# Zydak/Vulkan-Path-Tracer

Hardware: AMD Instinct MI355X
Metric: Msamples/s at 1920x1080 (higher is better)
Workload: dtype f32; 1 GPU; cornell_1080p_d8; scene=CornellBox (12 triangles, emissive quad 50), black env, width=1920, height=1080, max_depth=8, samples_per_frame=1, batches_per_gpu=14 x 904 frames, partition=rows y % N == rank, one ncclGather at the end, base_seed=1

## Files before the change

### vulkan-path-tracer_amd/_build.py

```python
import os
import subprocess
import sys

HERE = os.path.dirname(os.path.abspath(__file__))
CSRC = os.path.join(HERE, "csrc")
LIB = os.path.join(HERE, "libvpt_hip.so")
LIB_LAB = os.path.join(HERE, "libvpt_hip_lab.so")
SOURCES = ["kernels_whole.hip", "kernels_finish.hip", "kernels_bounce.hip", "kernels_aux.hip", "kernels_trace.hip", "kernels_stream.hip", "kernels_media.hip", "kernels_post.hip",
           "api_context.hip", "api_scene.hip", "api_render.hip", "api_post.hip", "api_comm.hip", "bvh_build.cpp"]
LAB_SOURCES = ["kernels_lab_r1.hip", "api_lab.hip"]
HEADERS = ["kernels_lut.hip", "device_types.hpp", "path_plan.hpp", "scene_prep.hpp", "grid_prep.hpp", "denoise.hpp", "temporal.hpp", "kernels.hpp", "api_ctx.hpp", "shading.hpp", "traverse.hpp", "bvh_build.hpp", "bvh_refit.hpp", "volume.hpp", "atmosphere.hpp", "wave.hpp", "shade_core.hpp", "vote.hpp", "slab.hpp", "whole_refill.hpp", "whole_args.hpp", "camera.hpp", "camera_cull.hpp",
           os.path.join("..", "..", "include", "vpt.h"), os.path.join("..", "..", "include", "vpt_lab.h"), os.path.join("..", "..", "include", "vpt_fp32.h")]
FLAGS = ["--offload-arch=gfx950", "-O3", "-std=c++17", "-fPIC", "-ffp-contract=off", "-fno-fast-math",
         "-fhip-fp32-correctly-rounded-divide-sqrt", "-Wno-unused-result", "-Wno-pass-failed"]
EXTRA_FLAGS = {f: ["-fno-slp-vectorize"] for f in ("kernels_trace.hip", "kernels_stream.hip", "kernels_media.hip", "kernels_whole.hip", "kernels_finish.hip", "kernels_bounce.hip", "kernels_aux.hip", "kernels_lab_r1.hip")}
EXTRA_FLAGS.update({f: ["-Os"] for f in ("api_context.hip", "api_scene.hip", "api_render.hip", "api_post.hip", "api_comm.hip")})
EXTRA_FLAGS["bvh_build.cpp"] = ["-O2"]
EXTRA_FLAGS["kernels_post.hip"] = ["-Xarch_host", "-Os"]


def hipcc():
    for c in (os.environ.get("HIPCC"), "/opt/rocm/bin/hipcc", "hipcc"):
        if c and (os.path.isabs(c) and os.path.exists(c) or not os.path.isabs(c)):
            return c
    raise RuntimeError("hipcc not found")


def _sources(lab):
    return SOURCES + (LAB_SOURCES if lab else [])


def source_id(defines=("-DVPT_LAB=0",)):
    import hashlib
    h = hashlib.sha256()
# ... 63 lines not shown
```

### vulkan-path-tracer_amd/csrc/api_context.hip

```cpp
#include <cmath>

#include "api_ctx.hpp"

using namespace vpt::api;

namespace {

bool media_on(const vpt_ctx* c) { return !c->volumes.empty() || c->dsc.atm_on; }
void free_path_buffers(Lane& L) {
    destroy_graph(L);
    if (L.ps_block) (void)hipFree(L.ps_block);
    L.ps_block = nullptr;
    if (L.ps_legacy) (void)hipFree(L.ps_legacy);
    L.ps_legacy = nullptr;
    for (int i = 0; i < 2; i++) { if (L.queue[i]) (void)hipFree(L.queue[i]); L.queue[i] = nullptr; }
    if (L.cqueue) (void)hipFree(L.cqueue);
    L.cqueue = nullptr;
    if (L.ss_block) (void)hipFree(L.ss_block);
    L.ss_block = nullptr;
    if (L.media_block) (void)hipFree(L.media_block);
    L.media_block = nullptr; L.ms = MediaState{}; L.media_frames = 0;
    for (uint32_t k = 0; k < kShadeClasses; k++) { if (L.class_queue[k]) (void)hipFree(L.class_queue[k]); L.class_queue[k] = nullptr; }
    if (L.cls_q) (void)hipFree(L.cls_q);
    L.cls_q = nullptr;
// ... 409 lines not shown
    free_render_buffers(c);
    if (c->d_launch_off) (void)hipFree(c->d_launch_off);
    if (c->d_volumes) (void)hipFree(c->d_volumes);
    for (DensityGrid& g : c->grids) { (void)hipFree((void*)g.values); (void)hipFree((void*)g.block_max); (void)hipFree((void*)g.bricks); }
    if (c->d_grids) (void)hipFree(c->d_grids);
    for (hipEvent_t e : c->ev_pool) (void)hipEventDestroy(e);
    lane_destroy(c->main);
    delete c;
}

const char* vpt_last_error(const vpt_ctx* c) { return c ? c->err.c_str() : "null context"; }

int vpt_set_camera(vpt_ctx* c, const float* vi, const float* pi) {
    if (!c || !vi || !pi) return VPT_ERR_INVALID_ARGUMENT;
    memcpy(c->P.view_inv, vi, 64); memcpy(c->P.proj_inv, pi, 64);
    c->state_gen++;
    reset_accum(c, true);
    return VPT_OK;
}

int vpt_set_params(vpt_ctx* c, const vpt_params* p) {
    if (!c || !p) return VPT_ERR_INVALID_ARGUMENT;
    if (p->samples_per_frame == 0 || p->samples_per_frame > 0xffffffu) return fail(c, VPT_ERR_INVALID_ARGUMENT, "samples_per_frame must be >= 1");
    if (p->max_depth == 0 || p->max_depth > 1000000u) return fail(c, VPT_ERR_INVALID_ARGUMENT, "max_depth must be in [1, 1000000]");
    if (p->screen_chunk_count == 0 || p->screen_chunk_count > 64) return fail(c, VPT_ERR_INVALID_ARGUMENT, "screen_chunk_count must be in [1, 64]");
    if (p->screen_chunk_count != 1 && c->P.shard_count != 1) return fail(c, VPT_ERR_UNSUPPORTED, "split-screen dispatch needs the whole image in one context (shard_count == 1): its first dispatch copies pixels across rows");
    {
        vpt_params same = *p; same.max_samples = c->params.max_samples;
        if (p->max_samples != c->params.max_samples && memcmp(&same, &c->params, sizeof(vpt_params)) == 0) { c->params.max_samples = p->max_samples; return VPT_OK; }
    }
    { int rd = drain(c); if (rd) return rd; }
    c->state_gen++;
    const bool flags_changed = c->params.flags != p->flags;
    c->dsc.strict_hits = (p->flags & VPT_FLAG_LOCAL_HITS) ? 1u : 0u;
    c->params = *p;
    sync_params(c);
    reset_accum(c);
    if (flags_changed && c->has_scene) {
        HIPCHK(c, hipSetDevice(c->cfg.device));
        int rc2 = refresh_material_tables(c); if (rc2) return rc2;
    }
    return VPT_OK;
}

int vpt_set_base_seed(vpt_ctx* c, uint32_t base_seed) {
    if (!c) return VPT_ERR_INVALID_ARGUMENT;
    { int rd = drain(c); if (rd) return rd; }
// ... 54 lines not shown
```

### vulkan-path-tracer_amd/csrc/api_render.hip

```cpp
#include "api_ctx.hpp"

using namespace vpt::api;
using plan::Kind;

namespace {


uint32_t split_dispatch_slots(const RenderParams& P, uint32_t dispatch) {
    const uint32_t S = P.split, ch = dispatch % (S * S), cx = ch % S, cy = ch / S;
    const uint32_t lw = cx < P.width ? (P.width - cx + S - 1) / S : 0, lh = cy < P.height ? (P.height - cy + S - 1) / S : 0;
    return lw * lh;
}
uint32_t batch_slots(const RenderParams& P, uint32_t frames, uint32_t dispatch_base) {
    if (P.split <= 1) return frames * P.shard_pixels;
    uint32_t n = 0;
    for (uint32_t k = 0; k < frames; k++) n += split_dispatch_slots(P, dispatch_base + k);
    return n;
}
int decide_batch(vpt_ctx* c, const Lane& L, const plan::Facts& f, uint32_t frames, uint32_t dispatch_base, bool capturing, plan::Schedule& sd) {
    if (frames == 0 || frames > L.frames_alloc) return fail(c, VPT_ERR_DEVICE, "internal: batch larger than the path buffers");
    sd = plan::decide(f, frames, L.frames_alloc, L.resident_alloc, batch_slots(c->P, frames, dispatch_base), &L != &c->main, capturing);
    return sd.err != VPT_OK ? fail(c, sd.err, sd.msg) : VPT_OK;
}
PathState part_state(const vpt_ctx* c, const Lane& L, uint32_t first_frame) {
    PathState ps = L.ps;
    const size_t at = (size_t)first_frame * c->P.shard_pixels;
    ps.ACC += at; ps.M += at; ps.maniso += at;
    return ps;
}
void resolve_part(vpt_ctx* c, Lane& L, const BatchState& b, uint32_t i, hipStream_t on) {
    const uint32_t first = b.sd.parts.first[i];
    const uint32_t* guard = plan::runs_fused(b.sd.kind) ? &L.ctr->alive3[b.k3] : plan::runs_streams(b.sd.kind) ? &L.sctr->alive[b.parity].v : &L.ctr->ray_count[b.parity];
    TIMED(c, on, VPT_K_RESOLVE, launch_resolve(on, c->P, part_state(c, L, first), c->image, b.sd.parts.first[i + 1] - first, b.dispatch_base + first, guard));
}
int batch_begin(vpt_ctx* c, Lane& L, const plan::Schedule& sd, uint32_t frames, uint32_t dispatch_base, Grids grids, BatchState& b) {
    hipStream_t s = L.stream;
    b = BatchState{};
    b.frames = frames; b.dispatch_base = dispatch_base; b.sd = sd;
    b.primary_grid = grids.primary; b.tail_grid = grids.tail;
    c->spill_dirty = true;
    const uint32_t n_slots = batch_slots(c->P, frames, dispatch_base);
    if (c->P.split > 1) {
        std::vector<uint32_t> off(frames + 1, 0u);
        for (uint32_t k = 0; k < frames; k++) off[k + 1] = off[k] + split_dispatch_slots(c->P, dispatch_base + k);
        HIPCHK(c, hipMemcpyAsync(c->d_launch_off, off.data(), off.size() * 4, hipMemcpyHostToDevice, s));
        HIPCHK(c, hipStreamSynchronize(s));
    }
    b.n_slots = n_slots;
    b.n_first = sd.regen ? sd.resident * c->P.shard_pixels : n_slots;
    b.count = c->cfg.count_traversal != 0;
    if (sd.kind == Kind::MediaStreams) {
        int rl = ensure_media_buffers(c, L); if (rl != VPT_OK) return rl;
        if (frames > L.media_frames) return fail(c, VPT_ERR_DEVICE, "internal: media batch larger than the media streams");
    }
    if (sd.kind == Kind::StagedR1) { int rl = ensure_legacy_buffers(c, L); if (rl != VPT_OK) return rl; }
    if (sd.kind == Kind::StreamsSorted) { int rl = ensure_sorted_buffers(c, L); if (rl != VPT_OK) return rl; }
    b.min_bounces = (uint64_t)c->P.max_depth * c->P.samples_per_frame;
    b.iter_cap = (b.min_bounces * 4ull + 1024ull) * ((frames + sd.resident - 1) / sd.resident);
    if (n_slots == 0) return VPT_OK;
    HIPCHK(c, hipMemsetAsync(L.ctr, 0, offsetof(Counters, stat_closest), s));
    const DeviceScene dsc = lane_scene(c, L);
    if (sd.kind == Kind::Whole) {
        b.parity = 1; b.k3 = 1; b.iter = 1;
        const cull::Packed rect = cull::pack(whole_cull_rect(c));
        for (uint32_t i = 0; i < sd.parts.n; i++) {
            const uint32_t first = sd.parts.first[i], n_part = sd.parts.n > 1u ? (sd.parts.first[i + 1] - first) * c->P.shard_pixels : n_slots;
            const uint32_t grid = std::max(1u, std::min<uint32_t>((uint32_t)std::min(c->whole_blocks, b.primary_grid), (n_part + 255u) / 256u));
            const uint32_t n_waves = grid * 4u, rounds = ((n_part + 63u) / 64u) / n_waves, mode = c->lab_whole_sched >> 4;
            const uint32_t static_rounds = (mode == 0u || mode == 3u) ? std::min(rounds, 1u) : mode == 1u ? (rounds >= 2u ? rounds - 1u : 0u) : rounds / 2u;
            if (i) HIPCHK(c, hipMemsetAsync(&L.ctr->extend_head, 0, 4, s));
            TIMED(c, s, VPT_K_PRIMARY, launch_whole(s, grid, b.count, dsc, c->P, part_state(c, L, first), L.ctr, n_part, dispatch_base + first, c->scene_plain, static_rounds, std::max(1u, c->lab_whole_sched & 15u) | (mode == 3u ? 0x100u : 0u), rect.x, rect.y));
            if (i + 1u < sd.parts.n) {
                HIPCHK(c, hipEventRecord(L.ev_shade, s));
                HIPCHK(c, hipStreamWaitEvent(L.stream2, L.ev_shade, 0));
                resolve_part(c, L, b, i, L.stream2);
            }
        }
    } else if (sd.kind == Kind::Fused) {
        TIMED(c, s, VPT_K_PRIMARY, launch_bounce(s, (uint32_t)b.primary_grid, c->lds_scene, b.count, true, dsc, c->P, L.ps, L.ss, nullptr, L.queue[1], L.ctr, 0u, b.n_first, dispatch_base, 0u, c->scene_plain));
        b.parity = 1; b.k3 = 1; b.iter = 1;
    } else if (plan::runs_streams(sd.kind)) {
        TIMED(c, s, VPT_K_PRIMARY, launch_raygen_stream(s, c->P, L.ps, L.ss, L.queue[0], b.n_first, dispatch_base, sd.kind == Kind::MediaStreams));
        launch_stream_begin(s, L.sctr, b.n_first, n_slots);
        b.parity = 0;
    } else {
#if VPT_LAB
        TIMED(c, s, VPT_K_PRIMARY, launch_raygen(s, c->P, L.ps, L.queue[0], L.ctr, n_slots, dispatch_base));
#endif
        b.parity = 0;
    }
    return VPT_OK;
}

int batch_bounces(vpt_ctx* c, Lane& L, BatchState& b, uint32_t bounces) {
// ... 509 lines not shown
```

### vulkan-path-tracer_amd/csrc/device_types.hpp

```cpp
#pragma once
#include <hip/hip_runtime.h>
#include <stdint.h>

#include "../../include/vpt.h"
#include "../../include/vpt_fp32.h"

namespace vpt {

using vptfp::V2;
using vptfp::V3;
using vptfp::V4;

struct BvhNode {
    float origin[3];
    float step_x;
    uint32_t lo[3];
    uint32_t hi[3];
    float step_y, step_z;
    int32_t child[4];
    __host__ __device__ void set_step(int axis, uint32_t biased_exponent) {
        uint32_t bits = biased_exponent << 23; float f; __builtin_memcpy(&f, &bits, 4);
        (axis == 0 ? step_x : axis == 1 ? step_y : step_z) = f;
    }
};
// ... 184 lines not shown
    uint32_t* SHI;
    float4* PE;
    float4* PS;
    float4* PL;
    float4* PT;
    float4* SKO;
    float4* SKD;
    float4* LTO;
    float4* LTD;
    unsigned char* vis_sky;
    unsigned char* vis_light;
    uint32_t cap;
};

struct MediaState {
    float4* MS;
    float4* MP[10];
};

struct alignas(256) HotWord {
    uint32_t v;
    uint32_t pad[63];
};
constexpr uint32_t kShadeMiss = 0, kShadePlain = 1, kShadeTextured = 2, kShadeGlass = 3, kShadeEmissive = 4, kShadeClasses = 5;
constexpr int kShadeAny = -1;

struct StreamCounters {
    HotWord queue_len[2];
    HotWord alive[2];
    HotWord pend_len, sky_len, light_len;
    HotWord extend_head, shade_head, sky_head, light_head;
    HotWord finish_head;
    HotWord class_len[kShadeClasses];
    HotWord class_head[kShadeClasses];
    uint32_t class_active[kShadeClasses];
    uint32_t class_exact[kShadeClasses];
    uint32_t class_base[kShadeClasses];
    uint32_t classify_done;
    uint32_t refill_next, refill_total;
    uint32_t refill_entry, refill_first, refill_count;
};

constexpr uint32_t kAppendChunk = 256;
constexpr uint32_t kAppendExactBelow = 1u << 21;
constexpr uint32_t kFusedExactBelow = kAppendExactBelow;

// ... 22 lines not shown
```

### vulkan-path-tracer_amd/csrc/kernels.hpp

```cpp
#pragma once
#include "device_types.hpp"
#include "denoise.hpp"
#include "temporal.hpp"
#include "../../include/vpt_lab.h"
#ifndef VPT_LAB
#define VPT_LAB 0
#endif

namespace vpt {

void launch_bounce(hipStream_t s, uint32_t blocks, bool lds_scene, bool count, bool first, const DeviceScene& sc, const RenderParams& P,
                   const PathState& ps, const StreamState& ss, const uint32_t* queue, uint32_t* queue_next, Counters* ctr, uint32_t parity, uint32_t n_slots,
                   uint32_t dispatch_base, uint32_t k3, bool plain = false);
int bounce_blocks_per_cu(bool lds_scene, const DeviceScene& sc, bool plain = false);
void launch_whole(hipStream_t s, uint32_t blocks, bool count, const DeviceScene& sc, const RenderParams& P, const PathState& ps, Counters* ctr, uint32_t n_slots,
                  uint32_t dispatch_base, bool plain, uint32_t static_rounds, uint32_t chunk_tiles, uint32_t cull_x, uint32_t cull_y);
int whole_blocks_per_cu(const DeviceScene& sc, bool plain);
void launch_finish(hipStream_t s, uint32_t blocks, bool count, const DeviceScene& sc, const RenderParams& P, const PathState& ps, const StreamState& ss, const uint32_t* queue,
                   StreamCounters* sctr, Counters* ctr, uint32_t parity);
int finish_blocks_per_cu(const DeviceScene& sc);
void launch_resolve(hipStream_t s, const RenderParams& P, const PathState& ps, float* image, uint32_t frames, uint32_t frame_base, const uint32_t* guard);
struct FirstHitArgs {
    const vpt_ray* rays; vpt_hit* hits; uint32_t n;
    uint32_t mode, frame;
    float* depth; uint4* ids; float4* normal; float4* albedo;
    float4* pick; uint32_t pixel;
};
void launch_first_hit(hipStream_t s, uint32_t blocks, const DeviceScene& sc, const RenderParams& P, const FirstHitArgs& a);
void launch_trace_rays(hipStream_t s, uint32_t blocks, const DeviceScene& sc, const vpt_ray* rays, uint32_t n, vpt_hit* hits);
void launch_read_density_grid(hipStream_t s, const DensityGrid& g, const int32_t* ijk, uint32_t n, float* out);
void launch_scatter_rows(hipStream_t s, const float* gathered, float* full, uint32_t w, uint32_t h, uint32_t shard_count, uint32_t stride_px);
void launch_precompute_materials(hipStream_t s, const DeviceScene& sc, uint32_t flags, MatResolved* out, uint32_t n);
void launch_precompute_tri_ng(hipStream_t s, const DeviceScene& sc, float4* out);
void launch_precompute_tri_shade(hipStream_t s, const DeviceScene& sc, float4* out);
void launch_precompute_emissive(hipStream_t s, const DeviceScene& sc, EmissiveTri* out, uint32_t total);
void launch_retransform_tris(hipStream_t s, const DeviceScene& sc, uint32_t total_tris, uint32_t n_inst, uint32_t first, uint32_t count, const float* xf, BvhTri* out, uint32_t* words);
void launch_refit_level(hipStream_t s, const DeviceScene& sc, const uint32_t* order, uint32_t begin, uint32_t end, const BvhTri* tris, float pad, float* boxes, BvhNode* nodes_out, BvhNodeWide* wide_out);
size_t traverse_lds_bytes(const DeviceScene& sc, bool lds_scene, int stack_rows);
size_t stack_overflow_bytes(uint32_t blocks);
// ... 94 lines not shown
```

### vulkan-path-tracer_amd/csrc/kernels_whole.hip

```cpp
#include "kernels.hpp"
#include "traverse.hpp"
#include "wave.hpp"
#include "shade_core.hpp"
#include "whole_refill.hpp"
#include "whole_args.hpp"
#include "camera_cull.hpp"

namespace vpt {

#define VPT_KERNARG __attribute__((address_space(4)))
template <> struct OneSampleFrames<VPT_KERNARG WholeParams> { static constexpr bool value = true; };

template <class Pm, class Ps>
__device__ __forceinline__ V3 whole_finish(const Pm& P, const Ps& ps, uint32_t slot, V3 E, V3 thr_prev, V3 light_prev, const ShadeOut& o) {
    const V3 light = light_prev + path_contribution(E, thr_prev, o.cflags, P.max_luminance);
    if (o.terminated) ps.ACC[slot] = finite3(light) ? f4(v3s(0.0f) + light, 0.0f) : make_float4(0.0f, 0.0f, 0.0f, 0.0f);
    return light;
}
template <bool COUNT, bool STRICT, bool PLAIN>
__global__ __launch_bounds__(kTraverseBlock, 3) void k_whole(WholeLaunch wl) {
    const WholeArgs& a = wl.a;
    const DeviceScene sc = a.sc;
    const RenderParams P = a.P;
    Counters* const ctr = a.ctr;
    extern __shared__ __align__(16) unsigned char smem[];
    const TravStackT<kWholeStackRows> stack = make_stack<kWholeStackRows>(smem, sc.stack_overflow);
    float4* lds_nodes = reinterpret_cast<float4*>(smem + kWholeStackRows * kTraverseBlock * 4);
    float4* lds_tris = lds_nodes + sc.node_count * 8;
    __shared__ CameraBlock cam;
    if (threadIdx.x == 0u) fill_camera_block(cam, P.view_inv, P.proj_inv, P.width, P.height, P.focus_distance, P.dof_strength);
    const VPT_KERNARG WholeArgs* ka = (const VPT_KERNARG WholeArgs*)__builtin_amdgcn_kernarg_segment_ptr();
    stage_scene<true>(sc, lds_nodes, lds_tris);
    constexpr uint32_t kWaves = kTraverseBlock / 64u;
    __shared__ uint32_t r_slot[kWaves][128], r_prim[kWaves][128], r_inst[kWaves][128];
    __shared__ float r_t[kWaves][128], r_u[kWaves][128], r_v[kWaves][128];
    __shared__ float4 r_ra[kWaves][128], r_rb[kWaves][128], r_rt[kWaves][128];
    __shared__ uint32_t f_slot[kWaves][refill::kTile], f_rng[kWaves][refill::kTile];
    __shared__ float f_ox[kWaves][refill::kTile], f_oy[kWaves][refill::kTile], f_oz[kWaves][refill::kTile];
    __shared__ float f_dx[kWaves][refill::kTile], f_dy[kWaves][refill::kTile], f_dz[kWaves][refill::kTile];
    const uint32_t wave = __builtin_amdgcn_readfirstlane(threadIdx.x >> 6);
    const refill::Shape shape{a.n_slots, gridDim.x * kWaves, a.static_rounds, a.chunk_tiles};
    refill::Cursor cur = refill::make_cursor(shape, blockIdx.x * kWaves + wave);
    refill::Fresh fresh = refill::make_fresh();
    uint32_t hit_head = 0u, hit_count = 0u;
    TravStats st, sst; st.nodes = 0; st.tris = 0; sst.nodes = 0; sst.tris = 0;
    uint32_t w_paths = 0u, w_rays = 0u, w_hits0 = 0u, w_alive0 = 0u, w_rays0 = 0u, w_parked = 0u;
#if VPT_LAB
    uint32_t w_culled = 0u;
#endif
    bool has_ray = false;
    uint32_t slot = 0u, rng_s = 0u, depth = 0u;
    bool in_medium = false;
    V3 porg = v3s(0.0f), pdir = v3s(0.0f), thr = v3s(1.0f), lightp = v3s(0.0f);
    float pdf = 1.0f;
    for (;;) {
        asm volatile("" : "+s"(ka));
        const VPT_KERNARG WholeScene<STRICT, PLAIN>& usc = static_cast<const VPT_KERNARG WholeScene<STRICT, PLAIN>&>(ka->sc);
        const VPT_KERNARG WholeParams& uP = static_cast<const VPT_KERNARG WholeParams&>(ka->P);
        const VPT_KERNARG PathState& ups = ka->ps;
        if (hit_count >= 64u || (refill::exhausted(cur, fresh) && hit_count > 0u)) {
            const uint32_t cnt = hit_count < 64u ? hit_count : 64u;
            const bool valid = lane_id() < cnt;
            uint32_t nrays = 0u;
            bool first = false, alive = false;
            if (valid) {
                const uint32_t q = (hit_head + lane_id()) & 127u;
                ShadeIn in_;
                const float4 a = r_ra[wave][q], b = r_rb[wave][q], t = r_rt[wave][q];
                slot = r_slot[wave][q];
                in_.rng = __float_as_uint(a.w);
                in_.porg = xyz(a); in_.pdir = xyz(b);
                const uint32_t dw = __float_as_uint(b.w);
// ... 30 lines not shown
            w_rays += (uint32_t)__popcll(__ballot(nrays >= 1u)) + (uint32_t)__popcll(__ballot(nrays >= 2u));
            w_rays0 += (uint32_t)__popcll(__ballot(first && nrays >= 1u)) + (uint32_t)__popcll(__ballot(first && nrays >= 2u));
            w_alive0 += (uint32_t)__popcll(__ballot(first && alive));
        }
        if (!refill::exhausted(cur, fresh)) {
#pragma unroll 1
            for (;;) {
                const unsigned long long m_free = __ballot(!has_ray);
                if (m_free == 0ull) break;
                if (fresh.count == 0u) {
                    if (refill::range_empty(cur) && !refill::take_static(shape, cur)) {
                        const uint32_t take = refill::dyn_take(shape, cur);
                        uint32_t k = 0u;
                        if (lane_id() == 0u) k = atomicAdd(&ctr->extend_head, take);
                        refill::take_dynamic(shape, cur, __builtin_amdgcn_readfirstlane(k), take);
                    }
                    if (refill::exhausted(cur, fresh)) break;
                    const uint32_t g = refill::gen_count(cur);
                    const uint32_t dispatch_base = uP.dispatch_base_dev ? *uP.dispatch_base_dev : ka->dispatch_base;
                    uint32_t gslot = 0u, x = 0u, y = 0u, f = 0u;
                    const VPT_KERNARG WholeLaunch* kl = (const VPT_KERNARG WholeLaunch*)ka;
                    const cull::Packed rect{kl->cull_x, kl->cull_y};
                    const bool bounded = !COUNT && (rect.x != cull::kAxisAll || rect.y != cull::kAxisAll);
                    bool keep = lane_id() < g;
                    if (keep) {
                        launch_pixel(uP, cur.w_next + lane_id(), dispatch_base, gslot, x, y, f);
                        if (bounded && cull::outside(rect, x, y)) {
                            keep = false;
                            ups.ACC[gslot] = make_float4(0.0f, 0.0f, 0.0f, 0.0f);
                        }
                    }
                    const unsigned long long m_keep = bounded ? __ballot(keep) : ~0ull >> (64u - g);
                    if (keep) {
                        const uint32_t seed = pcg_hash(uP.base_seed + dispatch_base + f);
                        Rng r; r.s = y + uP.width * x + seed;
                        V3 go, gd;
                        camera_ray(cam, r, x, y, go, gd);
                        const uint32_t j = bounded ? lanes_below(m_keep) : lane_id();
                        f_slot[wave][j] = gslot; f_rng[wave][j] = r.s;
                        f_ox[wave][j] = go.x; f_oy[wave][j] = go.y; f_oz[wave][j] = go.z;
                        f_dx[wave][j] = gd.x; f_dy[wave][j] = gd.y; f_dz[wave][j] = gd.z;
                    }
                    const uint32_t kept = (uint32_t)__popcll(m_keep);
                    w_paths += g - kept;
#if VPT_LAB
                    w_culled += g - kept;
#endif
                    refill::generated_kept(cur, fresh, g, kept);
                    __builtin_amdgcn_fence(__ATOMIC_RELEASE, "wavefront");
                    __builtin_amdgcn_wave_barrier();
                    __builtin_amdgcn_fence(__ATOMIC_ACQUIRE, "wavefront");
                    if (kept == 0u) continue;
                }
                const uint32_t q = fresh.head + lanes_below(m_free);
                refill::pop(fresh, (uint32_t)__popcll(m_free));
                if (!has_ray && q < fresh.head) {
                    slot = f_slot[wave][q]; rng_s = f_rng[wave][q];
                    porg = v3(f_ox[wave][q], f_oy[wave][q], f_oz[wave][q]);
                    pdir = v3(f_dx[wave][q], f_dy[wave][q], f_dz[wave][q]);
                    depth = 0u; in_medium = false; thr = v3s(1.0f); pdf = 1.0f; lightp = v3s(0.0f);
                    has_ray = true;
                }
            }
        }
        if (__ballot(has_ray) == 0ull) {
            if (refill::exhausted(cur, fresh) && hit_count == 0u) break;
            continue;
        }
        {
            HitRec hr;
            bool hit = false;
            if (has_ray) hit = trace_any<true, COUNT>(usc, lds_nodes, lds_tris, porg, normalize(pdir), 0.01f, 100000.0f, stack, hr, st);
            const unsigned long long mh = __ballot(has_ray && hit);
            if (has_ray && hit) {
                const uint32_t q = (hit_head + hit_count + lanes_below(mh)) & 127u;
// ... 10 lines not shown
            if (has_ray && !hit) {
                ShadeIn in_;
                in_.rng = rng_s; in_.porg = porg; in_.pdir = pdir; in_.depth = depth; in_.in_medium = in_medium; in_.thr_prev = thr; in_.prev_pdf = pdf;
                in_.vdepth = 0u; in_.cchan = -1; in_.vol_index = -1; in_.vol_t = 0.0f; in_.atm_comp = -1;
                in_.h = make_float4(-1.0f, 0.0f, 0.0f, 0.0f); in_.inst = 0u;
                ShadeOut o;
                shade_core<false, (int)kShadeMiss>(usc, uP, ups, slot, in_, o);
                (void)whole_finish(uP, ups, slot, o.emitted, thr, lightp, o);
            }
            has_ray = false;
            porg = v3s(0.0f); pdir = v3s(0.0f); thr = v3s(1.0f); lightp = v3s(0.0f); pdf = 1.0f; rng_s = 0u; depth = 0u; in_medium = false;
            __builtin_amdgcn_fence(__ATOMIC_RELEASE, "wavefront");
            __builtin_amdgcn_wave_barrier();
            __builtin_amdgcn_fence(__ATOMIC_ACQUIRE, "wavefront");
        }
    }
    if (lane_id() == 0) {
        if (w_paths) atomicAdd(&ctr->stat_closest, (unsigned long long)w_paths);
        if (w_rays) atomicAdd(&ctr->stat_shadow, (unsigned long long)w_rays);
        if (w_hits0) atomicAdd(&ctr->stat_primary_hits, (unsigned long long)w_hits0);
        if (w_alive0) atomicAdd(&ctr->stat_primary_alive, (unsigned long long)w_alive0);
        if (w_rays0) atomicAdd(&ctr->stat_primary_rays, (unsigned long long)w_rays0);
        if (w_parked) atomicAdd(&ctr->stat_connect, (unsigned long long)w_parked);
#if VPT_LAB
        if (w_culled) atomicAdd(&ctr->whole_culled, w_culled);
#endif
    }
    if (COUNT) {
        atomicAdd(&ctr->stat_nodes, (unsigned long long)st.nodes);
        atomicAdd(&ctr->stat_tris, (unsigned long long)st.tris);
        atomicAdd(&ctr->stat_shadow_nodes, (unsigned long long)sst.nodes);
        atomicAdd(&ctr->stat_shadow_tris, (unsigned long long)sst.tris);
    }
}

void launch_whole(hipStream_t s, uint32_t blocks, bool count, const DeviceScene& sc, const RenderParams& P, const PathState& ps, Counters* ctr, uint32_t n_slots,
                  uint32_t dispatch_base, bool plain, uint32_t static_rounds, uint32_t chunk_tiles, uint32_t cull_x, uint32_t cull_y) {
    const size_t lds = traverse_lds_bytes(sc, true, kWholeStackRows);
    const dim3 g(blocks), b(kTraverseBlock);
    void (*k)(WholeLaunch);
    if (plain && !count && !sc.strict_hits && sc.env_black) k = k_whole<false, false, true>;
    else if (sc.strict_hits) k = count ? k_whole<true, true, false> : k_whole<false, true, false>;
    else k = count ? k_whole<true, false, false> : k_whole<false, false, false>;
    hipLaunchKernelGGL(k, g, b, lds, s, WholeLaunch{WholeArgs{sc, P, ps, ctr, n_slots, dispatch_base, static_rounds, chunk_tiles}, cull_x, cull_y});
}
int whole_blocks_per_cu(const DeviceScene& sc, bool plain) {
    int nb = 0;
    const size_t lds = traverse_lds_bytes(sc, true, kWholeStackRows);
    if (plain) (void)hipOccupancyMaxActiveBlocksPerMultiprocessor(&nb, k_whole<false, false, true>, kTraverseBlock, lds);
    else (void)hipOccupancyMaxActiveBlocksPerMultiprocessor(&nb, k_whole<false, false, false>, kTraverseBlock, lds);
    return nb > 0 ? nb : 1;
}

}
```

### vulkan-path-tracer_amd/csrc/shade_core.hpp

```cpp
#pragma once
#include "shading.hpp"
#include "volume.hpp"
#include "atmosphere.hpp"
#include "wave.hpp"

namespace vpt {

__device__ inline float4 f4(V3 v, float w) { return make_float4(v.x, v.y, v.z, w); }
__device__ inline float4 f4u(V3 v, uint32_t w) { return make_float4(v.x, v.y, v.z, __uint_as_float(w)); }
__device__ inline V3 xyz(float4 v) { return v3(v.x, v.y, v.z); }
__device__ __forceinline__ V3 path_contribution(V3 E, V3 thr_prev, uint32_t cflags, float max_luminance) {
    V3 contrib = E * thr_prev;
    if (cflags & kCF_Clamp) {
        float lum = dot(contrib, v3(0.212671f, 0.715160f, 0.072169f));
        contrib = contrib * (max_luminance / max_(lum, max_luminance));
    }
    return contrib;
}
__device__ __forceinline__ bool finite3(V3 v) { return !isinf_(v.x) && !isinf_(v.y) && !isinf_(v.z) && !isnan_(v.x) && !isnan_(v.y) && !isnan_(v.z); }
template <class Pm>
__device__ inline void pixel_of_slot(const Pm& P, uint32_t slot, uint32_t& x, uint32_t& y, uint32_t& f) {
    f = slot / P.shard_pixels;
    uint32_t sp = slot - f * P.shard_pixels;
    uint32_t ys = sp / P.width;
// ... 144 lines not shown
            else {
                float att = VPT_C_MIE_ABSORPTION / VPT_C_MIE;
                bxdf = v3s(phase_mie(pdir, nd) * att); new_pdf = phase_hg(pdir, nd, 0.85f);
            }
        }
        new_d = nd;
        new_depth = depth + 1u;
    } else if (VOL && msc->atm_on && h.x < 0.0f) {
        new_depth = kMaxDepthMarker;
    } else if (CLS == kShadeMiss || (CLS == kShadeAny && h.x < 0.0f)) {
        V4 cp = v4(0.0f, 0.0f, 0.0f, 1.0f);
        if (((P.flags & VPT_FLAG_SHOW_ENV_DIRECTLY) || depth > 0) && sc.env_black) {
            cp = v4(0.0f, 0.0f, 0.0f, 0.0f);
        } else if ((P.flags & VPT_FLAG_SHOW_ENV_DIRECTLY) || depth > 0) {
            V3 d = rotate_sc(pdir, v3(1.0f, 0.0f, 0.0f), P.sky_rot[4], P.sky_rot[5]);
            d = rotate_sc(d, v3(0.0f, 1.0f, 0.0f), P.sky_rot[6], P.sky_rot[7]);
            V2 uv = direction_to_uv(d);
            cp = env_sample(sc, uv.x, uv.y);
        }
        emitted = v3(cp.x, cp.y, cp.z) * P.sky_intensity;
        if (P.flags & VPT_FLAG_FURNACE) emitted = v3s(1.0f);
        if ((P.flags & VPT_FLAG_SKY_MIS) && depth > 0) emitted = emitted * power_heuristics(prev_pdf, cp.w);
        new_depth = kMaxDepthMarker;
    } else {
        V3 rd = normalize(pdir);
        uint32_t inst_id = in_.inst;
        const InstanceDesc& in = sc.instances[inst_id];
        const vpt_material& mat = sc.materials[in.material];
        MatResolved mr = sc.mat_resolved[in.material];
        if (CLS == (int)kShadePlain || sc.all_plain) mr.flags = 63u;
        const bool geo_only = (P.flags & VPT_FLAG_GEOMETRY_NORMALS) != 0;
        SurfaceFrame s;
        surface_geom(sc, s, in, __float_as_uint(h.w), h.y, h.z, rd, geo_only);
        MatTaps taps;
        material_issue(sc.texels, mr, s.uv, geo_only, taps);
        surface_frame(s, rd, geo_only, mr, taps.normal);
        Bsdf bs; V3 mcol; float mdens, maniso, arot;
        bsdf_init(bs, sc, mat, mr, taps, s.inside, P.flags, mcol, mdens, maniso, arot);
        bool is_light = bs.emissive.x > 0.0f || bs.emissive.y > 0.0f || bs.emissive.z > 0.0f;
        rotate_tangents(s, mr.rot_sin, mr.rot_cos);
        bool scattered = false;
        if (in_medium) {
            float pm_aniso = ps.maniso[slot];
            if (pm_aniso != 1.0f) {
                float4 m = ps.M[slot];
                float gd = length(porg - s.pos);
// ... 177 lines not shown
```

### vulkan-path-tracer_amd/csrc/whole_args.hpp

```cpp
#pragma once
#include <stddef.h>

#include "device_types.hpp"

namespace vpt {

struct WholeArgs {
    DeviceScene sc;
    RenderParams P;
    PathState ps;
    Counters* ctr;
    uint32_t n_slots, dispatch_base;
    uint32_t static_rounds, chunk_tiles;
};

struct WholeLaunch {
    WholeArgs a;
    uint32_t cull_x, cull_y;
};
static_assert(offsetof(WholeLaunch, a) == 0, "the loop reads the argument segment as a WholeArgs");

template <bool STRICT, bool PLAIN>
struct WholeScene : DeviceScene {
    static constexpr uint32_t strict_hits = STRICT ? 1u : 0u, all_plain = 0u;
};
template <bool STRICT>
struct WholeScene<STRICT, true> : DeviceScene {
    static constexpr uint32_t strict_hits = STRICT ? 1u : 0u, all_plain = 1u, env_black = 1u;
};
struct WholeParams : RenderParams {
    static constexpr uint32_t samples_per_frame = 1u;
};
static_assert(sizeof(WholeScene<false, false>) == sizeof(DeviceScene) && sizeof(WholeScene<true, true>) == sizeof(DeviceScene) && sizeof(WholeParams) == sizeof(RenderParams),
              "the views add no word");

}
```

### vulkan-path-tracer_amd/csrc/whole_refill.hpp

```cpp
#pragma once
#include <stdint.h>

#include "../../include/vpt_fp32.h"

namespace vpt {
namespace refill {

constexpr uint32_t kTile = 64u;

struct Shape {
    uint32_t n;
    uint32_t n_waves;
    uint32_t static_rounds;
    uint32_t chunk_tiles;
};
VPT_HD uint32_t n_tiles(const Shape& s) { return (s.n + kTile - 1u) / kTile; }
VPT_HD uint32_t dyn_first(const Shape& s) { return s.static_rounds * s.n_waves; }

struct Cursor {
    uint32_t next_static;
    uint32_t w_next, w_end;
    uint32_t last_seen;
    bool done;
};
// ... 13 lines not shown
    const uint32_t tile = c.next_static;
    c.next_static += s.n_waves;
    set_range(s, c, tile, 1u);
    return true;
}
VPT_HD uint32_t dyn_take(const Shape& s, const Cursor& c) {
    uint32_t take = s.chunk_tiles & 0xffu;
    if (s.chunk_tiles & 0x100u) {
        const uint32_t left_tiles = n_tiles(s) > c.last_seen ? n_tiles(s) - c.last_seen : 0u, fair = left_tiles / (2u * s.n_waves);
        take = fair < 1u ? 1u : (fair < take ? fair : take);
    }
    return take;
}
VPT_HD void take_dynamic(const Shape& s, Cursor& c, uint32_t counter_before, uint32_t take) {
    const uint32_t tile = dyn_first(s) + counter_before;
    c.last_seen = tile + take;
    set_range(s, c, tile, take);
}

struct Fresh { uint32_t head, count; };
VPT_HD Fresh make_fresh() { Fresh f; f.head = 0u; f.count = 0u; return f; }
VPT_HD uint32_t gen_count(const Cursor& c) { const uint32_t left = c.w_end - c.w_next; return left < kTile ? left : kTile; }
VPT_HD void generated(Cursor& c, Fresh& f, uint32_t g) { c.w_next += g; f.head = 0u; f.count = g; }
VPT_HD void generated_kept(Cursor& c, Fresh& f, uint32_t g, uint32_t kept) { c.w_next += g; f.head = 0u; f.count = kept; }
VPT_HD uint32_t pop(Fresh& f, uint32_t want) {
    const uint32_t k = want < f.count ? want : f.count;
    f.head += k; f.count -= k;
    return k;
}
VPT_HD bool exhausted(const Cursor& c, const Fresh& f) { return c.done && f.count == 0u; }

}
}
```

Measured before the change: 10140 Msamples/s.

## Deal only camera-visible pixels to whole-kernel waves instead of culling per lane

Instead of launching every pixel slot and discarding those outside the camera cull rectangle per lane, the host computes a compact deal of only in-rectangle pixels per shard (and per split chunk), and the whole kernel decodes launch indices directly into rectangle pixels. Accumulator entries for culled pixels are zeroed in bulk runs after row ends or by a memset, and culled counts are reported once by the host-supplied value. A miss with one-sample frames now terminates early in the shade core. This removes the wasted lanes and ballot compaction for culled pixels, at the cost of more index arithmetic and extra zeroing passes; for a Cornell box that may already fill the screen, the rectangle may cover everything, so the new path may not activate.

```diff
diff --git a/vulkan-path-tracer_amd/_build.py b/vulkan-path-tracer_amd/_build.py
--- a/vulkan-path-tracer_amd/_build.py
+++ b/vulkan-path-tracer_amd/_build.py
@@ -9,7 +9,7 @@
 SOURCES = ["kernels_whole.hip", "kernels_finish.hip", "kernels_bounce.hip", "kernels_aux.hip", "kernels_trace.hip", "kernels_stream.hip", "kernels_media.hip", "kernels_post.hip",
            "api_context.hip", "api_scene.hip", "api_render.hip", "api_post.hip", "api_comm.hip", "bvh_build.cpp"]
 LAB_SOURCES = ["kernels_lab_r1.hip", "api_lab.hip"]
-HEADERS = ["kernels_lut.hip", "device_types.hpp", "path_plan.hpp", "scene_prep.hpp", "grid_prep.hpp", "denoise.hpp", "temporal.hpp", "kernels.hpp", "api_ctx.hpp", "shading.hpp", "traverse.hpp", "bvh_build.hpp", "bvh_refit.hpp", "volume.hpp", "atmosphere.hpp", "wave.hpp", "shade_core.hpp", "vote.hpp", "slab.hpp", "whole_refill.hpp", "whole_args.hpp", "camera.hpp", "camera_cull.hpp",
+HEADERS = ["kernels_lut.hip", "device_types.hpp", "path_plan.hpp", "scene_prep.hpp", "grid_prep.hpp", "denoise.hpp", "temporal.hpp", "kernels.hpp", "api_ctx.hpp", "shading.hpp", "traverse.hpp", "bvh_build.hpp", "bvh_refit.hpp", "volume.hpp", "atmosphere.hpp", "wave.hpp", "shade_core.hpp", "vote.hpp", "slab.hpp", "whole_refill.hpp", "whole_args.hpp", "whole_deal.hpp", "camera.hpp", "camera_cull.hpp",
            os.path.join("..", "..", "include", "vpt.h"), os.path.join("..", "..", "include", "vpt_lab.h"), os.path.join("..", "..", "include", "vpt_fp32.h")]
 FLAGS = ["--offload-arch=gfx950", "-O3", "-std=c++17", "-fPIC", "-ffp-contract=off", "-fno-fast-math",
          "-fhip-fp32-correctly-rounded-divide-sqrt", "-Wno-unused-result", "-Wno-pass-failed"]
diff --git a/vulkan-path-tracer_amd/csrc/api_context.hip b/vulkan-path-tracer_amd/csrc/api_context.hip
--- a/vulkan-path-tracer_amd/csrc/api_context.hip
+++ b/vulkan-path-tracer_amd/csrc/api_context.hip
@@ -455,7 +455,7 @@
 int vpt_set_params(vpt_ctx* c, const vpt_params* p) {
     if (!c || !p) return VPT_ERR_INVALID_ARGUMENT;
     if (p->samples_per_frame == 0 || p->samples_per_frame > 0xffffffu) return fail(c, VPT_ERR_INVALID_ARGUMENT, "samples_per_frame must be >= 1");
-    if (p->max_depth == 0 || p->max_depth > 1000000u) return fail(c, VPT_ERR_INVALID_ARGUMENT, "max_depth must be in [1, 1000000]");
+    if (p->max_depth == 0 || p->max_depth > kMaxDepthLimit) return fail(c, VPT_ERR_INVALID_ARGUMENT, "max_depth must be in [1, 1000000]");
     if (p->screen_chunk_count == 0 || p->screen_chunk_count > 64) return fail(c, VPT_ERR_INVALID_ARGUMENT, "screen_chunk_count must be in [1, 64]");
     if (p->screen_chunk_count != 1 && c->P.shard_count != 1) return fail(c, VPT_ERR_UNSUPPORTED, "split-screen dispatch needs the whole image in one context (shard_count == 1): its first dispatch copies pixels across rows");
     {
diff --git a/vulkan-path-tracer_amd/csrc/api_render.hip b/vulkan-path-tracer_amd/csrc/api_render.hip
--- a/vulkan-path-tracer_amd/csrc/api_render.hip
+++ b/vulkan-path-tracer_amd/csrc/api_render.hip
@@ -40,9 +40,13 @@
     b.primary_grid = grids.primary; b.tail_grid = grids.tail;
     c->spill_dirty = true;
     const uint32_t n_slots = batch_slots(c->P, frames, dispatch_base);
+    const cull::Rect wrect = sd.kind == Kind::Whole ? whole_cull_rect(c) : cull::everything(c->P.width, c->P.height);
+    uint32_t n_split_dealt = 0;
     if (c->P.split > 1) {
         std::vector<uint32_t> off(frames + 1, 0u);
-        for (uint32_t k = 0; k < frames; k++) off[k + 1] = off[k] + split_dispatch_slots(c->P, dispatch_base + k);
+        for (uint32_t k = 0; k < frames; k++)
+            off[k + 1] = off[k] + (wrect.all ? split_dispatch_slots(c->P, dispatch_base + k) : deal::split_rect_px(wrect, (dispatch_base + k) % (c->P.split * c->P.split), c->P.split));
+        n_split_dealt = off[frames];
         HIPCHK(c, hipMemcpyAsync(c->d_launch_off, off.data(), off.size() * 4, hipMemcpyHostToDevice, s));
         HIPCHK(c, hipStreamSynchronize(s));
     }
@@ -62,14 +66,20 @@
     const DeviceScene dsc = lane_scene(c, L);
     if (sd.kind == Kind::Whole) {
         b.parity = 1; b.k3 = 1; b.iter = 1;
-        const cull::Packed rect = cull::pack(whole_cull_rect(c));
+        const bool dealt = !wrect.all, split = c->P.split > 1;
+        const cull::Packed rect = cull::pack(wrect);
         for (uint32_t i = 0; i < sd.parts.n; i++) {
-            const uint32_t first = sd.parts.first[i], n_part = sd.parts.n > 1u ? (sd.parts.first[i + 1] - first) * c->P.shard_pixels : n_slots;
+            const uint32_t first = sd.parts.first[i], part_frames = sd.parts.n > 1u ? sd.parts.first[i + 1] - first : frames;
+            const uint32_t part_slots = sd.parts.n > 1u ? part_frames * c->P.shard_pixels : n_slots;
+            const deal::Deal dl = dealt ? deal::make(wrect, c->P.shard_rank, c->P.shard_count, c->P.width, part_slots) : deal::Deal{};
+            const uint32_t n_part = !dealt ? part_slots : split ? n_split_dealt : part_frames * dl.rect_px;
+            const uint64_t culled = part_slots - n_part;
+            if (dealt && (n_part == 0u || split)) HIPCHK(c, hipMemsetAsync(part_state(c, L, first).ACC, 0, (size_t)(split ? frames * c->P.shard_pixels : part_slots) * 16, s));
             const uint32_t grid = std::max(1u, std::min<uint32_t>((uint32_t)std::min(c->whole_blocks, b.primary_grid), (n_part + 255u) / 256u));
             const uint32_t n_waves = grid * 4u, rounds = ((n_part + 63u) / 64u) / n_waves, mode = c->lab_whole_sched >> 4;
             const uint32_t static_rounds = (mode == 0u || mode == 3u) ? std::min(rounds, 1u) : mode == 1u ? (rounds >= 2u ? rounds - 1u : 0u) : rounds / 2u;
             if (i) HIPCHK(c, hipMemsetAsync(&L.ctr->extend_head, 0, 4, s));
-            TIMED(c, s, VPT_K_PRIMARY, launch_whole(s, grid, b.count, dsc, c->P, part_state(c, L, first), L.ctr, n_part, dispatch_base + first, c->scene_plain, static_rounds, std::max(1u, c->lab_whole_sched & 15u) | (mode == 3u ? 0x100u : 0u), rect.x, rect.y));
+            TIMED(c, s, VPT_K_PRIMARY, launch_whole(s, grid, b.count, dsc, c->P, part_state(c, L, first), L.ctr, n_part, dispatch_base + first, c->scene_plain, static_rounds, std::max(1u, c->lab_whole_sched & 15u) | (mode == 3u ? 0x100u : 0u), rect, dl, culled));
             if (i + 1u < sd.parts.n) {
                 HIPCHK(c, hipEventRecord(L.ev_shade, s));
                 HIPCHK(c, hipStreamWaitEvent(L.stream2, L.ev_shade, 0));
diff --git a/vulkan-path-tracer_amd/csrc/device_types.hpp b/vulkan-path-tracer_amd/csrc/device_types.hpp
--- a/vulkan-path-tracer_amd/csrc/device_types.hpp
+++ b/vulkan-path-tracer_amd/csrc/device_types.hpp
@@ -230,6 +230,7 @@
     uint32_t v;
     uint32_t pad[63];
 };
+constexpr uint32_t kMaxDepthLimit = 1000000u;
 constexpr uint32_t kShadeMiss = 0, kShadePlain = 1, kShadeTextured = 2, kShadeGlass = 3, kShadeEmissive = 4, kShadeClasses = 5;
 constexpr int kShadeAny = -1;
 
diff --git a/vulkan-path-tracer_amd/csrc/kernels.hpp b/vulkan-path-tracer_amd/csrc/kernels.hpp
--- a/vulkan-path-tracer_amd/csrc/kernels.hpp
+++ b/vulkan-path-tracer_amd/csrc/kernels.hpp
@@ -2,6 +2,7 @@
 #include "device_types.hpp"
 #include "denoise.hpp"
 #include "temporal.hpp"
+#include "whole_deal.hpp"
 #include "../../include/vpt_lab.h"
 #ifndef VPT_LAB
 #define VPT_LAB 0
@@ -14,7 +15,7 @@
                    uint32_t dispatch_base, uint32_t k3, bool plain = false);
 int bounce_blocks_per_cu(bool lds_scene, const DeviceScene& sc, bool plain = false);
 void launch_whole(hipStream_t s, uint32_t blocks, bool count, const DeviceScene& sc, const RenderParams& P, const PathState& ps, Counters* ctr, uint32_t n_slots,
-                  uint32_t dispatch_base, bool plain, uint32_t static_rounds, uint32_t chunk_tiles, uint32_t cull_x, uint32_t cull_y);
+                  uint32_t dispatch_base, bool plain, uint32_t static_rounds, uint32_t chunk_tiles, cull::Packed rect, const deal::Deal& deal, uint64_t culled);
 int whole_blocks_per_cu(const DeviceScene& sc, bool plain);
 void launch_finish(hipStream_t s, uint32_t blocks, bool count, const DeviceScene& sc, const RenderParams& P, const PathState& ps, const StreamState& ss, const uint32_t* queue,
                    StreamCounters* sctr, Counters* ctr, uint32_t parity);
diff --git a/vulkan-path-tracer_amd/csrc/kernels_whole.hip b/vulkan-path-tracer_amd/csrc/kernels_whole.hip
--- a/vulkan-path-tracer_amd/csrc/kernels_whole.hip
+++ b/vulkan-path-tracer_amd/csrc/kernels_whole.hip
@@ -17,6 +17,10 @@
     if (o.terminated) ps.ACC[slot] = finite3(light) ? f4(v3s(0.0f) + light, 0.0f) : make_float4(0.0f, 0.0f, 0.0f, 0.0f);
     return light;
 }
+__device__ __attribute__((noinline)) void whole_zero_run(float4* acc, uint32_t first, uint32_t end) {
+    for (uint32_t i = first + lane_id(); i < end; i += 64u) acc[i] = make_float4(0.0f, 0.0f, 0.0f, 0.0f);
+}
+
 template <bool COUNT, bool STRICT, bool PLAIN>
 __global__ __launch_bounds__(kTraverseBlock, 3) void k_whole(WholeLaunch wl) {
     const WholeArgs& a = wl.a;
@@ -45,9 +49,6 @@
     uint32_t hit_head = 0u, hit_count = 0u;
     TravStats st, sst; st.nodes = 0; st.tris = 0; sst.nodes = 0; sst.tris = 0;
     uint32_t w_paths = 0u, w_rays = 0u, w_hits0 = 0u, w_alive0 = 0u, w_rays0 = 0u, w_parked = 0u;
-#if VPT_LAB
-    uint32_t w_culled = 0u;
-#endif
     bool has_ray = false;
     uint32_t slot = 0u, rng_s = 0u, depth = 0u;
     bool in_medium = false;
@@ -124,35 +125,46 @@
                     const VPT_KERNARG WholeLaunch* kl = (const VPT_KERNARG WholeLaunch*)ka;
                     const cull::Packed rect{kl->cull_x, kl->cull_y};
                     const bool bounded = !COUNT && (rect.x != cull::kAxisAll || rect.y != cull::kAxisAll);
-                    bool keep = lane_id() < g;
-                    if (keep) {
-                        launch_pixel(uP, cur.w_next + lane_id(), dispatch_base, gslot, x, y, f);
-                        if (bounded && cull::outside(rect, x, y)) {
-                            keep = false;
-                            ups.ACC[gslot] = make_float4(0.0f, 0.0f, 0.0f, 0.0f);
-                        }
-                    }
-                    const unsigned long long m_keep = bounded ? __ballot(keep) : ~0ull >> (64u - g);
-                    if (keep) {
+                    bool row_end = false, at_frame_end = false;
+                    if (lane_id() < g) {
+                        const uint32_t li = cur.w_next + lane_id();
+                        if (uP.split != 1u) {
+                            const uint32_t x0 = bounded ? cull::axis_first(rect.x) : 0u, y0 = bounded ? cull::axis_first(rect.y) : 0u;
+                            deal::decode_split(x0, bounded ? x0 + cull::axis_span(rect.x) : uP.width - 1u, y0, bounded ? y0 + cull::axis_span(rect.y) : uP.height - 1u,
+                                               uP.split, uP.width, uP.shard_pixels, uP.launch_off, dispatch_base, li, gslot, x, y, f);
+                        } else if (bounded) {
+                            const deal::Deal d{kl->deal.x0, kl->deal.rw, kl->deal.ys0, kl->deal.rect_px, 0u, kl->deal.last_in_frame, 0u, 0u};
+                            deal::decode(d, uP.shard_pixels, uP.width, uP.shard_rank, uP.shard_count, li, gslot, x, y, f);
+                            row_end = x == kl->deal.x0 + kl->deal.rw - 1u; at_frame_end = deal::frame_end(d, uP.shard_pixels, f, gslot);
+                        } else { gslot = li; pixel_of_slot(uP, li, x, y, f); }
                         const uint32_t seed = pcg_hash(uP.base_seed + dispatch_base + f);
                         Rng r; r.s = y + uP.width * x + seed;
                         V3 go, gd;
                         camera_ray(cam, r, x, y, go, gd);
-                        const uint32_t j = bounded ? lanes_below(m_keep) : lane_id();
+                        const uint32_t j = lane_id();
                         f_slot[wave][j] = gslot; f_rng[wave][j] = r.s;
                         f_ox[wave][j] = go.x; f_oy[wave][j] = go.y; f_oz[wave][j] = go.z;
                         f_dx[wave][j] = gd.x; f_dy[wave][j] = gd.y; f_dz[wave][j] = gd.z;
                     }
-                    const uint32_t kept = (uint32_t)__popcll(m_keep);
-                    w_paths += g - kept;
-#if VPT_LAB
-                    w_culled += g - kept;
-#endif
-                    refill::generated_kept(cur, fresh, g, kept);
+                    const bool first_tile = cur.w_next == 0u;
+                    refill::generated(cur, fresh, g);
                     __builtin_amdgcn_fence(__ATOMIC_RELEASE, "wavefront");
                     __builtin_amdgcn_wave_barrier();
                     __builtin_amdgcn_fence(__ATOMIC_ACQUIRE, "wavefront");
-                    if (kept == 0u) continue;
+                    if (bounded && uP.split == 1u) {
+                        unsigned long long m_end = __ballot(row_end);
+                        const unsigned long long m_last = __ballot(at_frame_end);
+                        if (first_tile)
+                            whole_zero_run(ups.ACC, 0u, kl->deal.head);
+                        const deal::Deal dz{kl->deal.x0, kl->deal.rw, kl->deal.ys0, kl->deal.rect_px, kl->deal.gap, kl->deal.last_in_frame, kl->deal.head, kl->deal.slots};
+                        while (m_end != 0ull) {
+                            const uint32_t b = (uint32_t)__builtin_ctzll(m_end);
+                            uint32_t first, end;
+                            deal::run_after(dz, uP.shard_pixels, __builtin_amdgcn_readfirstlane(f_slot[wave][b]), ((m_last >> b) & 1ull) != 0ull, first, end);
+                            m_end &= m_end - 1ull;
+                            whole_zero_run(ups.ACC, first, end);
+                        }
+                    }
                 }
                 const uint32_t q = fresh.head + lanes_below(m_free);
                 refill::pop(fresh, (uint32_t)__popcll(m_free));
@@ -209,9 +221,15 @@
         if (w_alive0) atomicAdd(&ctr->stat_primary_alive, (unsigned long long)w_alive0);
         if (w_rays0) atomicAdd(&ctr->stat_primary_rays, (unsigned long long)w_rays0);
         if (w_parked) atomicAdd(&ctr->stat_connect, (unsigned long long)w_parked);
+    }
+    if (!COUNT && blockIdx.x == 0u && threadIdx.x == 0u) {
+        const unsigned long long culled = ((const VPT_KERNARG WholeLaunch*)ka)->culled;
+        if (culled) {
+            atomicAdd(&ctr->stat_closest, culled);
 #if VPT_LAB
-        if (w_culled) atomicAdd(&ctr->whole_culled, w_culled);
+            atomicAdd(&ctr->whole_culled, (uint32_t)culled);
 #endif
+        }
     }
     if (COUNT) {
         atomicAdd(&ctr->stat_nodes, (unsigned long long)st.nodes);
@@ -222,14 +240,14 @@
 }
 
 void launch_whole(hipStream_t s, uint32_t blocks, bool count, const DeviceScene& sc, const RenderParams& P, const PathState& ps, Counters* ctr, uint32_t n_slots,
-                  uint32_t dispatch_base, bool plain, uint32_t static_rounds, uint32_t chunk_tiles, uint32_t cull_x, uint32_t cull_y) {
+                  uint32_t dispatch_base, bool plain, uint32_t static_rounds, uint32_t chunk_tiles, cull::Packed rect, const deal::Deal& deal, uint64_t culled) {
     const size_t lds = traverse_lds_bytes(sc, true, kWholeStackRows);
     const dim3 g(blocks), b(kTraverseBlock);
     void (*k)(WholeLaunch);
     if (plain && !count && !sc.strict_hits && sc.env_black) k = k_whole<false, false, true>;
     else if (sc.strict_hits) k = count ? k_whole<true, true, false> : k_whole<false, true, false>;
     else k = count ? k_whole<true, false, false> : k_whole<false, false, false>;
-    hipLaunchKernelGGL(k, g, b, lds, s, WholeLaunch{WholeArgs{sc, P, ps, ctr, n_slots, dispatch_base, static_rounds, chunk_tiles}, cull_x, cull_y});
+    hipLaunchKernelGGL(k, g, b, lds, s, WholeLaunch{WholeArgs{sc, P, ps, ctr, n_slots, dispatch_base, static_rounds, chunk_tiles}, rect.x, rect.y, deal, culled});
 }
 int whole_blocks_per_cu(const DeviceScene& sc, bool plain) {
     int nb = 0;
diff --git a/vulkan-path-tracer_amd/csrc/shade_core.hpp b/vulkan-path-tracer_amd/csrc/shade_core.hpp
--- a/vulkan-path-tracer_amd/csrc/shade_core.hpp
+++ b/vulkan-path-tracer_amd/csrc/shade_core.hpp
@@ -190,6 +190,11 @@
         if (P.flags & VPT_FLAG_FURNACE) emitted = v3s(1.0f);
         if ((P.flags & VPT_FLAG_SKY_MIS) && depth > 0) emitted = emitted * power_heuristics(prev_pdf, cp.w);
         new_depth = kMaxDepthMarker;
+        if constexpr (!VOL && CLS == (int)kShadeMiss && OneSampleFrames<Pm>::value) {
+            static_assert(kMaxDepthLimit <= kMaxDepthMarker, "a miss must end its path whatever max_depth is");
+            out.alive = false; out.terminated = true; out.cflags = kCF_Clamp | kCF_Finalize; out.emitted = emitted;
+            return;
+        }
     } else {
         V3 rd = normalize(pdir);
         uint32_t inst_id = in_.inst;
diff --git a/vulkan-path-tracer_amd/csrc/whole_args.hpp b/vulkan-path-tracer_amd/csrc/whole_args.hpp
--- a/vulkan-path-tracer_amd/csrc/whole_args.hpp
+++ b/vulkan-path-tracer_amd/csrc/whole_args.hpp
@@ -2,6 +2,7 @@
 #include <stddef.h>
 
 #include "device_types.hpp"
+#include "whole_deal.hpp"
 
 namespace vpt {
 
@@ -17,6 +18,8 @@
 struct WholeLaunch {
     WholeArgs a;
     uint32_t cull_x, cull_y;
+    deal::Deal deal;
+    unsigned long long culled;
 };
 static_assert(offsetof(WholeLaunch, a) == 0, "the loop reads the argument segment as a WholeArgs");
 
diff --git a/vulkan-path-tracer_amd/csrc/whole_deal.hpp b/vulkan-path-tracer_amd/csrc/whole_deal.hpp
--- /dev/null
+++ b/vulkan-path-tracer_amd/csrc/whole_deal.hpp
@@ -0,0 +1,62 @@
+#pragma once
+#include <stdint.h>
+
+#include "camera_cull.hpp"
+
+namespace vpt {
+namespace deal {
+
+struct Deal { uint32_t x0, rw, ys0, rect_px, gap, last_in_frame, head, slots; };
+VPT_HD void shard_rows(uint32_t first, uint32_t last, uint32_t shard_rank, uint32_t shard_count, uint32_t& ys0, uint32_t& rh) {
+    ys0 = first > shard_rank ? (first - shard_rank + shard_count - 1u) / shard_count : 0u;
+    rh = 0u;
+    if (first > last || last < shard_rank) return;
+    const uint32_t ys1 = (last - shard_rank) / shard_count;
+    if (ys1 >= ys0) rh = ys1 - ys0 + 1u;
+}
+VPT_HD Deal make(const cull::Rect& r, uint32_t shard_rank, uint32_t shard_count, uint32_t width, uint32_t slots) {
+    Deal d; d.x0 = r.x0; d.rw = 0u; d.ys0 = 0u; d.rect_px = 0u; d.gap = 0u; d.last_in_frame = 0u; d.head = 0u; d.slots = slots;
+    uint32_t rh = 0u;
+    if (r.x0 <= r.x1 && r.y0 <= r.y1) { d.rw = r.x1 - r.x0 + 1u; shard_rows(r.y0, r.y1, shard_rank, shard_count, d.ys0, rh); }
+    d.rect_px = d.rw * rh;
+    if (d.rect_px != 0u) { d.gap = width - d.rw; d.head = d.ys0 * width + d.x0; d.last_in_frame = (d.ys0 + rh - 1u) * width + d.x0 + d.rw - 1u; }
+    return d;
+}
+VPT_HD void decode(const Deal& d, uint32_t shard_pixels, uint32_t width, uint32_t shard_rank, uint32_t shard_count, uint32_t li,
+                   uint32_t& slot, uint32_t& x, uint32_t& y, uint32_t& f) {
+    f = li / d.rect_px;
+    const uint32_t r = li - f * d.rect_px, ry = r / d.rw, ys = d.ys0 + ry;
+    x = d.x0 + r - ry * d.rw;
+    y = shard_rank + shard_count * ys;
+    slot = f * shard_pixels + ys * width + x;
+}
+VPT_HD bool frame_end(const Deal& d, uint32_t shard_pixels, uint32_t f, uint32_t slot) { return slot - f * shard_pixels == d.last_in_frame; }
+VPT_HD void run_after(const Deal& d, uint32_t shard_pixels, uint32_t slot, bool at_frame_end, uint32_t& first, uint32_t& end) {
+    first = slot + 1u;
+    if (!at_frame_end) { end = first + d.gap; return; }
+    const uint32_t next = slot - d.last_in_frame + shard_pixels + d.head;
+    end = next < d.slots ? next : d.slots;
+}
+VPT_HD uint64_t culled(uint32_t frames, uint32_t shard_pixels, uint32_t rect_px) { return (uint64_t)frames * (shard_pixels - rect_px); }
+
+VPT_HD void split_axis(uint32_t first, uint32_t last, uint32_t c, uint32_t S, uint32_t& l0, uint32_t& n) { shard_rows(first, last, c, S, l0, n); }
+VPT_HD uint32_t split_rect_px(const cull::Rect& r, uint32_t chunk, uint32_t S) {
+    uint32_t lx0, lw, ly0, lh;
+    split_axis(r.x0, r.x1, chunk % S, S, lx0, lw); split_axis(r.y0, r.y1, chunk / S, S, ly0, lh);
+    return lw * lh;
+}
+template <class Off>
+VPT_HD void decode_split(uint32_t x0, uint32_t x1, uint32_t y0, uint32_t y1, uint32_t S, uint32_t width, uint32_t shard_pixels, const Off& off, uint32_t dispatch_base,
+                         uint32_t li, uint32_t& slot, uint32_t& x, uint32_t& y, uint32_t& f) {
+    uint32_t k = 0u;
+    while (off[k + 1u] <= li) k++;
+    const uint32_t r = li - off[k], c = (dispatch_base + k) % (S * S), cx = c % S, cy = c / S;
+    uint32_t lx0, lw, ly0, lh;
+    split_axis(x0, x1, cx, S, lx0, lw); split_axis(y0, y1, cy, S, ly0, lh);
+    const uint32_t ly = r / lw, lx = r - ly * lw;
+    x = (lx0 + lx) * S + cx; y = (ly0 + ly) * S + cy; f = k;
+    slot = k * shard_pixels + y * width + x;
+}
+
+}
+}
diff --git a/vulkan-path-tracer_amd/csrc/whole_refill.hpp b/vulkan-path-tracer_amd/csrc/whole_refill.hpp
--- a/vulkan-path-tracer_amd/csrc/whole_refill.hpp
+++ b/vulkan-path-tracer_amd/csrc/whole_refill.hpp
@@ -59,7 +59,6 @@
 VPT_HD Fresh make_fresh() { Fresh f; f.head = 0u; f.count = 0u; return f; }
 VPT_HD uint32_t gen_count(const Cursor& c) { const uint32_t left = c.w_end - c.w_next; return left < kTile ? left : kTile; }
 VPT_HD void generated(Cursor& c, Fresh& f, uint32_t g) { c.w_next += g; f.head = 0u; f.count = g; }
-VPT_HD void generated_kept(Cursor& c, Fresh& f, uint32_t g, uint32_t kept) { c.w_next += g; f.head = 0u; f.count = kept; }
 VPT_HD uint32_t pop(Fresh& f, uint32_t want) {
     const uint32_t k = want < f.count ? want : f.count;
     f.head += k; f.count -= k;
```

Result: faster. 10480 Msamples/s (median of 6 runs) (+3.3%).
